# fkluger/vanishing_points_2017

Measured on AMD Instinct MI355X. Metric: images/sec (LSD->CNN->EM) + horizon-AUC parity, YUD-shape, 1/2/4/8 GPU, higher is better.
Workload: dtype f32 (CNN: f32 operands / accumulation / results; conv1 multiply EXACT bf16 pieces of the f32 operands (three per operand) on the bf16 matrix cores; conv2-5, fc6 and fc7 multiply scaled fp16 PAIRS of the f32 operands (22 of 24 significand bits, three exact products per f32 product) on the fp16 matrix

## Files before the change

### __graft_entry__.py

```python
import os
import subprocess
import sys

ROOT = os.path.dirname(os.path.abspath(__file__))
if ROOT not in sys.path:
    sys.path.insert(0, ROOT)


def build():
    from vanishing_points_2017_amd import build as vbuild
    so = vbuild.build(verbose=True)
    sim = os.path.join(ROOT, "tests", "hostsim")
    out = os.path.join(sim, "_build")
    os.makedirs(out, exist_ok=True)
    subprocess.check_call(["g++", "-O2", "-std=c++17", "-ffp-contract=off", "-fPIC", "-shared",
                           "-Wno-unknown-pragmas", os.path.join(sim, "sim_em.cpp"), "-o",
                           os.path.join(out, "libvpk_hostsim.so")])
    subprocess.check_call(["g++", "-O2", "-std=c++17", "-ffp-contract=off", "-fPIC", "-shared",
                           os.path.join(sim, "sim_raster.cpp"), "-o", os.path.join(out, "libvpk_hostsim_raster.so")])
    subprocess.check_call(["g++", "-O2", "-std=c++17", "-Wall", "-Werror", "-fPIC", "-shared",
                           os.path.join(sim, "sim_cnn_plan.cpp"), "-o", os.path.join(out, "libvpk_hostsim_cnn_plan.so")])
    odir = os.path.join(ROOT, "oracle", "_build")
    os.makedirs(odir, exist_ok=True)
    subprocess.check_call(["gcc", "-O2", "-fPIC", "-shared", "-ffp-contract=off", "-fno-builtin",
                           os.path.join(ROOT, "oracle", "_fma.c"), "-o", os.path.join(odir, "libvpkfma.so"), "-lm"])
    import vanishing_points_2017_amd
    from vanishing_points_2017_amd import _lib
    lib = _lib.load()
    missing = [s for s in _lib.EXPORTS if not hasattr(lib, s)]
    if missing:
        raise RuntimeError("libvpk.so lacks symbols: %s" % missing)
    print("built", so)


def smoke():
    import numpy as np
    import torch
    assert torch.cuda.is_available(), "smoke() needs cuda:0"
    from vanishing_points_2017_amd import synth, vp_localisation
    from oracle import em_numpy
    from oracle import agg_raster
    from vanishing_points_2017_amd import sphere_mapping
    sc = synth.make_scene(4242, 90, 3)
    ln = sc["l"]
    sc["sphere_image"] = sphere_mapping.sphere_line_plot(ln.copy(), 500, alpha=0.1)
    assert np.array_equal(sc["sphere_image"], agg_raster.raster(ln)), "the sphere raster differs from the oracle"
    got = vp_localisation.expectation_maximisation(sc["l"].copy(), sc["lp"].copy(), sc["cnn_response"],
                                                   sphere_image=sc["sphere_image"])
    ref = em_numpy.expectation_maximisation(sc["l"].copy(), sc["lp"].copy(), sc["cnn_response"].copy(),
                                            sphere_image=sc["sphere_image"])
    assert np.array_equal(got["vp_assoc"], ref["vp_assoc"]), "line->VP assignments differ from the oracle"
    assert np.abs(got["vp"] - ref["vp"]).max() < 1e-4
    from oracle import cnn_torch
    from vanishing_points_2017_amd import cnn
    w, mean = cnn.synthetic_weights(0), cnn.synthetic_mean(0)
    sphere = sc["sphere_image"][None]
    want = cnn_torch.forward(w, mean, sphere)
    net = cnn.Net(w, mean)
    err = []
    for alg in (4, 2):
        net.set_algorithm(alg)
        err.append(float(np.abs(net.forward(sphere) - want).max()))
    net.set_algorithm(4)
    assert max(err) <= 2e-5, "CNN response differs from the oracle: %s" % err
    print("smoke ok: raster of %d lines exact; %d VPs, %d iterations; CNN max |diff| %.1e (default: fp16 pairs) / %.1e (exact bf16 triples + Winograd f32)" % (
        ln.shape[0], got["vp"].shape[0], got["iterations"], err[0], err[1]))


if __name__ == "__main__":
    build()
    if len(sys.argv) > 1 and sys.argv[1] == "smoke":
        smoke()
```

### vanishing_points_2017_amd/cnn.py

```python
import ctypes

import numpy as np

from ._lib import VPK_ERR_RANGE, VpkRangeError
from .runtime import get_runtime

LAYER_SHAPES = [
    ("conv1", (96, 1, 11, 11)), ("conv2", (256, 48, 5, 5)), ("conv3", (384, 256, 3, 3)),
    ("conv4", (384, 192, 3, 3)), ("conv5", (256, 192, 3, 3)), ("fc6", (4096, 57600)),
    ("fc7", (4096, 4096)), ("fc8", (400, 4096)),
]
RANGE_POLICIES = {"raise": 0, "recompute_exact": 1}


def range_policy_code(policy):
    if policy not in RANGE_POLICIES:
        raise ValueError("range policy must be one of %s, got %r" % (sorted(RANGE_POLICIES), policy))
    return RANGE_POLICIES[policy]


FLOAT_DTYPES = ("float16", "float32", "float64")


def image_kind(images):
# ... 51 lines not shown
            if w.shape != shape or b.shape != (shape[0],):
                raise ValueError("%s: expected weight %s / bias (%d,), got %s / %s" % (name, shape, shape[0], w.shape, b.shape))
            keep += [w, b]
            blobs += [w.ctypes.data, b.ctypes.data]
        mean = np.ascontiguousarray(np.asarray(mean, dtype=np.float32).reshape(500, 500))
        arr = (ctypes.c_void_p * 16)(*blobs)
        self.rt.check(self.rt.lib.vpk_cnn_load(self.rt.h, arr, ctypes.c_void_p(mean.ctypes.data)))
        self._last_batch = None

    def forward_device(self, sphere, tap=None):
        f32 = image_kind(sphere) == "f32"
        if f32 and len(sphere.shape) != 3:
            raise ValueError("forward_device: float images must be (B, 500, 500), got shape %s" % (tuple(sphere.shape),))
        rt = self.rt
        t = rt.torch
        batch = int(sphere.shape[0])
        if f32 and sphere.is_cuda:
            rt.stream.wait_stream(t.cuda.current_stream(sphere.device))
        with rt.on_stream():
            if f32:
                sphere = sphere.to(device=rt.tdev, dtype=t.float32).contiguous()
            out = t.empty((batch, 20, 20), dtype=t.float32, device=rt.tdev)
            if tap is None:
                fwd = rt.lib.vpk_cnn_forward_f32 if f32 else rt.lib.vpk_cnn_forward
                rt.check(fwd(rt.h, rt.ptr(sphere), batch, rt.ptr(out)))
                self._last_batch = batch
                return out
            tp = t.empty((batch,) + TAP_SHAPES[tap], dtype=t.float32, device=rt.tdev)
            fwd = rt.lib.vpk_cnn_forward_tap_f32 if f32 else rt.lib.vpk_cnn_forward_tap
            rt.check(fwd(rt.h, rt.ptr(sphere), batch, rt.ptr(out), int(tap), rt.ptr(tp)))
            return out, tp

    LAYER_NAMES = ["conv1", "norm1", "pool1", "conv2", "norm2", "pool2", "conv3", "conv4", "conv5", "pool5",
                   "fc6", "fc7", "fc8"]
    LAYER_FLOP = {"conv1": 2 * 96 * 15129 * 121, "conv2": 2 * 256 * 3721 * 1200, "conv3": 2 * 384 * 900 * 2304,
                  "conv4": 2 * 384 * 900 * 1728, "conv5": 2 * 256 * 900 * 1728, "fc6": 2 * 57600 * 4096,
                  "fc7": 2 * 4096 * 4096, "fc8": 2 * 4096 * 400}

    @classmethod
    def executed_flop(cls, layer, fusion=3, precision=0, algorithm=4, batch=102):
        alg = cls.LAYER_FLOP[layer]
        if layer == "conv1":
            if fusion == 3:
                return 168 * 12 * 72 * 2.0 * 16 * 16 * 32, "bf16"
            if fusion == 4:
                return 168 * 12 * 48 * 2.0 * 16 * 16 * 32, "f16"
            if fusion == 1:
                return 168 * 8 * 186 * 2.0 * 16 * 16 * 4, "f32"
            return alg * 128.0 / 121.0, "f32"
        if layer in ("conv2", "conv3", "conv4", "conv5"):
            if precision == 1:
                return 6.0 * alg, "bf16"
            if algorithm == 4:
                tiles, steps = {"conv2": (2 * 16 * 2 * 1, 75), "conv3": (1 * 8 * 1 * 3, 16 * 9), "conv4": (2 * 4 * 1 * 3, 12 * 9),
                                "conv5": (2 * 8 * 1 * 1, 12 * 9)}[layer]
                return tiles * steps * 4 * 12 * 2.0 * 32 * 32 * 16, "f16"
            if layer == "conv2" and algorithm >= 2:
                return 64 * 4 * 75 * 24 * 2.0 * 32 * 32 * 16, "bf16"
            if algorithm >= 1:
                return alg * (36.0 / 100.0 if layer == "conv2" else 16.0 / 36.0), "f32"
            return alg, "f32"
        pad = (-(-batch // 128) * 128) / float(batch)
        if precision == 0 and ((layer == "fc6" and algorithm >= 2) or (layer == "fc7" and algorithm == 4)):
            return alg * pad * (3.0 if algorithm == 4 else 6.0), "f16" if algorithm == 4 else "bf16"
        return alg * pad, "f32"

    def set_fusion(self, on=3):
        self.rt.check(self.rt.lib.vpk_cnn_set_fusion(self.rt.h, int(on)))

    def set_algorithm(self, mode):
        self.rt.check(self.rt.lib.vpk_cnn_set_algorithm(self.rt.h, int(mode)))

    def set_precision(self, mode):
        self.rt.check(self.rt.lib.vpk_cnn_set_precision(self.rt.h, int(mode)))

    RANGE_LAYERS = ["conv2", "conv3", "conv4", "conv5", "fc6", "fc7"]

    def activation_scales(self):
        sc = (ctypes.c_float * 6)()
        self.rt.check(self.rt.lib.vpk_cnn_get_activation_scales(self.rt.h, sc))
        return np.array([float(x) for x in sc], dtype=np.float32)

    def set_activation_scales(self, scales):
        sc = (ctypes.c_float * 6)(*[float(x) for x in scales])
        self.rt.check(self.rt.lib.vpk_cnn_set_activation_scales(self.rt.h, sc))

    def calibrate(self, rasters=None):
        rt = self.rt
        if rasters is None:
            rt.check(rt.lib.vpk_cnn_calibrate(rt.h, None, 0))
            return
        t = rt.torch
        if not isinstance(rasters, t.Tensor):
            rasters = t.from_numpy(np.ascontiguousarray(rasters, dtype=np.uint8).reshape(-1, 500, 500))
        with rt.on_stream():
            d = rasters.to(rt.tdev).contiguous()
        rt.synchronize()
        rt.check(rt.lib.vpk_cnn_calibrate(rt.h, rt.ptr(d), int(d.shape[0])))

    def range_flags(self):
        w = ctypes.c_uint32(0)
        rc = self.rt.lib.vpk_cnn_range_flags(self.rt.h, ctypes.byref(w))
        if rc not in (0, VPK_ERR_RANGE):
            self.rt.check(rc)
        return int(w.value)

    def check_range(self):
        w = ctypes.c_uint32(0)
        rc = self.rt.lib.vpk_cnn_range_flags(self.rt.h, ctypes.byref(w))
# ... 94 lines not shown
```

### vanishing_points_2017_amd/csrc/cnn_conv_pieces.hpp

```cpp
#ifndef VPK_CNN_CONV_PIECES_HPP_
#define VPK_CNN_CONV_PIECES_HPP_

namespace {

constexpr int CP_THREADS = 256;
constexpr int CP_TC = 32;

struct PieceDims {
    int B;
    int Cg16, CGtot, Hp, Wp;
    int OC, OH, OW, groups;
    int KW, ntaps, ksteps;
    int mblocks;
    int mtiles, rtiles, ctiles;
    int relu;
    int OHp, OWp, opad;
    long long in_image;
    int o_cgtot, o_Hp, o_Wp, o_pad;
    float o_ascale;
    unsigned* range_word;
    unsigned range_bit;
    unsigned* img_range;
    const int* live;
    float oscale;
};


template <int NP>
__global__ __launch_bounds__(256) void to_planes_kernel(const float* __restrict__ in, unsigned short* __restrict__ out, int C, int Hp,
                                                        int Wp, float ascale, unsigned* __restrict__ range_word, unsigned range_bit,
                                                        unsigned* __restrict__ img_range, const int* __restrict__ live) {
    const int y = blockIdx.x, cg = blockIdx.y, b = blockIdx.z;
    if (live && b >= *live) return;
    const float* src = in + (((size_t)b * C + cg * 16) * Hp + y) * Wp;
    u32x4* dst = reinterpret_cast<u32x4*>(out) + (((size_t)b * (C >> 4) + cg) * (2 * NP) * Hp + y) * Wp;
    bool bad = false;
    for (int idx = threadIdx.x; idx < 2 * Wp; idx += 256) {
        const int h = idx / Wp, x = idx - h * Wp;
        unsigned short p[3][8];
#pragma unroll
        for (int e = 0; e < 8; ++e) {
            const float v = src[(size_t)(8 * h + e) * Hp * Wp + x];
            if (NP == 3) split3(v, p[0][e], p[1][e], p[2][e]);
            else split2h_guard(v * ascale, p[0][e], p[1][e], bad);
        }
#pragma unroll
        for (int q = 0; q < NP; ++q) {
            u32x4 w4;
#pragma unroll
            for (int e = 0; e < 4; ++e) w4[e] = (unsigned)p[q][2 * e] | ((unsigned)p[q][2 * e + 1] << 16);
            dst[(size_t)(2 * q + h) * Hp * Wp + x] = w4;
        }
    }
    if (NP == 2) range_report(bad, range_word, range_bit, img_range ? img_range + b : nullptr);
}

template <int N>
__device__ __forceinline__ void cp_wait() {
    asm volatile("s_waitcnt vmcnt(%0)" ::"n"(N) : "memory");
    __builtin_amdgcn_sched_barrier(0);
}

template <int OFF>
__device__ __forceinline__ void cp_gload16(bf16x8& dst, const void* sbase, unsigned voff) {
    asm volatile("global_load_dwordx4 %0, %1, %2 offset:%3" : "+v"(dst) : "v"(voff), "s"(sbase), "n"(OFF) : "memory");
}

template <int KH, int NB, int NP, int RH>
__global__ __launch_bounds__(CP_THREADS, 2) void conv_pieces_kernel(PieceDims d, const unsigned short* __restrict__ act,
                                                                     const unsigned short* __restrict__ wfrag,
                                                                     const float* __restrict__ bias, float* __restrict__ out,
                                                                     unsigned short* __restrict__ out_planes,
                                                                     int* __restrict__ tile_counter, int total_tiles) {
    constexpr int MB = 4 / RH;
    constexpr int TR = RH * NB;
    constexpr int PR = TR + KH - 1, PC = CP_TC + KH - 1;
    constexpr int KPP = (PC + 7) / 8;
    constexpr int PARTS = PR > 8 ? 2 : 1;
    constexpr int GST = (PR > 8 ? PR * 128 : 1024) + 128;
    static_assert(GST % 256 == 128, "odd multiple of 128 bytes");
    if (d.live) {
        d.B = __builtin_amdgcn_readfirstlane(*d.live);
        total_tiles = d.groups * d.B * d.rtiles * d.ctiles * d.mtiles;
    }
    constexpr int PLANE = KPP * GST;
    constexpr int NPL = 2 * NP;
    constexpr int PBUF = NPL * PLANE;
    constexpr int NDMA = NPL * KPP * PARTS;
    constexpr int NPW = (NDMA + 3) / 4;
    constexpr int NPR = NP == 3 ? 6 : 3;
    constexpr int NSETS = NP == 3 ? 2 : (KH == 5 ? 5 : (RH == 2 ? 6 : 3));
    constexpr int D = NSETS;
    constexpr int KHB = KH == 5 ? 5 : 1;
    constexpr int FP = KH == 5 ? 5 : 9;
    constexpr int NPWB = (NPW + KHB - 1) / KHB;
    static_assert(PR <= 16 && NB == 4 && (RH == 1 || RH == 2) && KH * KH == KHB * FP && (NP == 2 || NP == 3), "8 row slots per DMA instruction; two halves");
    __shared__ __attribute__((aligned(16))) unsigned char cp_lds[2 * PBUF];
    __shared__ int s_next[2];
    const int tid = threadIdx.x, lane = tid & 63;
    const int wave = __builtin_amdgcn_readfirstlane(tid >> 6);
    const int wmq = RH == 1 ? wave : (wave & 1);
    const int rh = RH == 1 ? 0 : (wave >> 1);
    const int n31 = lane & 31, kh_ = lane >> 5;
    const unsigned lds0 = lds_addr(cp_lds);
    typedef __attribute__((address_space(3))) const bf16x8 lds_cbf8;
    unsigned vb[KH];
#pragma unroll
    for (int kw = 0; kw < KH; ++kw) {
        const unsigned c = (unsigned)(n31 + kw);
        vb[kw] = lds0 + (unsigned)(kh_ * PLANE + rh * NB * 128) + (c >> 3) * (unsigned)GST + (c & 7u) * 16u;
    }
    const unsigned voff_a = (unsigned)lane * 16u;
    int parity = 0;
    for (int tile = blockIdx.x; tile < total_tiles;) {
        int nx = 0;
        if (tid == 0)
            asm volatile("s_nop 4\n\tglobal_atomic_add %0, %1, %2, %3 sc0" : "=v"(nx) : "v"(0), "v"(1), "s"(tile_counter) : "memory");
        int t = tile;
        const int mt = t % d.mtiles; t /= d.mtiles;
        const int ct = t % d.ctiles; t /= d.ctiles;
        const int rt = t % d.rtiles; t /= d.rtiles;
        const int b = t % d.B;
        const int g = t / d.B;
        const int y0 = rt * TR, x0 = ct * CP_TC;
        const unsigned char* in_g = reinterpret_cast<const unsigned char*>(act) + (size_t)b * d.in_image +
                                    (size_t)g * d.Cg16 * NPL * d.Hp * d.Wp * 16;
        const size_t plane_bytes = (size_t)d.Hp * d.Wp * 16;
        const int yr = y0 + (lane >> 3) < d.Hp ? y0 + (lane >> 3) : d.Hp - 1;
        const unsigned voff_p = (unsigned)(yr * d.Wp + x0 + (lane & 7)) * 16u;
        const int yr2 = y0 + 8 + (lane >> 3) < d.Hp ? y0 + 8 + (lane >> 3) : d.Hp - 1;
        const unsigned voff_p2 = (unsigned)(yr2 * d.Wp + x0 + (lane & 7)) * 16u;
        auto issue_dma = [&](int cg, int k) __attribute__((always_inline)) {
            int q = wave * NPW + k;
            q = q < NDMA ? q : NDMA - 1;
            const int part = q / (NPL * KPP), q1 = q - part * (NPL * KPP);
            const int pl = q1 / KPP, kk = q1 - pl * KPP;
            const unsigned char* src = in_g + ((size_t)cg * NPL + pl) * plane_bytes + (size_t)kk * 128;
            const unsigned dst = lds0 + (unsigned)((cg & 1) * PBUF + pl * PLANE + kk * GST);
            if (PARTS == 1 || part == 0) dma16(voff_p, src, __builtin_amdgcn_readfirstlane(dst));
            else if (lane < 8 * (PR - 8)) dma16(voff_p2, src, __builtin_amdgcn_readfirstlane(dst + 1024u));
        };
        const unsigned char* wgrp = reinterpret_cast<const unsigned char*>(wfrag) +
                                    ((size_t)g * d.ksteps * d.mblocks + (size_t)mt * MB + wmq) * NP * 1024;
        const unsigned wstep = (unsigned)d.mblocks * NP * 1024;
        bf16x8 af[NSETS][NP], bfr[NB][NP];
#pragma unroll
        for (int q = 0; q < NSETS * NP; ++q) af[q / NP][q % NP] = __builtin_bit_cast(bf16x8, u32x4{0u, 0u, 0u, 0u});
        auto load_a = [&](const unsigned char* src, auto o_tag) __attribute__((always_inline)) {
            constexpr int o = decltype(o_tag)::value;
            cp_gload16<0>(af[o][0], src, voff_a);
            cp_gload16<1024>(af[o][1], src, voff_a);
            if constexpr (NP == 3) cp_gload16<2048>(af[o][2], src, voff_a);
        };
        auto fetch_b = [&](auto row_tag, auto k_tag, unsigned va) __attribute__((always_inline)) {
            constexpr int j = decltype(row_tag)::value, k = decltype(k_tag)::value;
            constexpr int dkh = KH == 5 ? 0 : k / KH;
#pragma unroll
            for (int p = 0; p < NP; ++p) bfr[j][p] = *(lds_cbf8*)(va + (unsigned)((j + dkh) * 128 + p * 2 * PLANE));
        };
        auto tap_address = [&](auto k_tag, unsigned sb) __attribute__((always_inline)) {
            constexpr int k = decltype(k_tag)::value;
            return vb[KH == 5 ? k : k % KH] + sb;
        };
        auto fetch_all = [&](auto k_tag, unsigned sb) __attribute__((always_inline)) {
            const unsigned va = tap_address(k_tag, sb);
            fetch_b(std::integral_constant<int, 0>(), k_tag, va); fetch_b(std::integral_constant<int, 1>(), k_tag, va);
            fetch_b(std::integral_constant<int, 2>(), k_tag, va); fetch_b(std::integral_constant<int, 3>(), k_tag, va);
        };
        f32x2v acc[NB][8];
        f32x16 tq[NB];
#pragma unroll
        for (int j = 0; j < NB; ++j) {
#pragma unroll
            for (int e = 0; e < 8; ++e) acc[j][e] = f32x2v{0.f, 0.f};
#pragma unroll
            for (int e = 0; e < 16; ++e) tq[j][e] = 0.f;
        }
        const int S = d.ksteps;
        __builtin_amdgcn_s_barrier();
#pragma unroll
        for (int k = 0; k < NPW; ++k) issue_dma(0, k);
        asm volatile("s_nop 4" ::: "memory");
        load_a(wgrp, std::integral_constant<int, 0>());
        load_a(wgrp + wstep, std::integral_constant<int, 1>());
        if constexpr (NSETS > 2) load_a(wgrp + 2 * wstep, std::integral_constant<int, 2>());
        if constexpr (NSETS > 3) { load_a(wgrp + 3 * wstep, std::integral_constant<int, 3>()); load_a(wgrp + 4 * wstep, std::integral_constant<int, 4>()); }
        if constexpr (NSETS > 5) load_a(wgrp + 5 * wstep, std::integral_constant<int, 5>());
        const unsigned char* anext = wgrp + (size_t)D * wstep;
        cp_wait<0>();
        if (tid == 0) s_next[parity] = nx + (int)gridDim.x;
        asm volatile("s_waitcnt lgkmcnt(0)" ::: "memory");
        __builtin_amdgcn_s_barrier();
        fetch_all(std::integral_constant<int, 0>(), 0u);
        auto products = [&](auto o_tag, auto row_tag, auto first_tag) __attribute__((always_inline)) {
            constexpr int o = decltype(o_tag)::value, j = decltype(row_tag)::value;
            constexpr bool first = decltype(first_tag)::value;
            constexpr int PA[6] = {NP == 3 ? 2 : 1, NP == 3 ? 1 : 0, 0, 1, 0, 0}, PB[6] = {0, 1, NP == 3 ? 2 : 0, 0, 1, 0};
            const f32x16 zero = {0.f, 0.f, 0.f, 0.f, 0.f, 0.f, 0.f, 0.f, 0.f, 0.f, 0.f, 0.f, 0.f, 0.f, 0.f, 0.f};
#pragma unroll
            for (int p = 0; p < NPR; ++p) {
                if constexpr (NP == 3)
                    tq[j] = __builtin_amdgcn_mfma_f32_32x32x16_bf16(af[o][PA[p]], bfr[j][PB[p]], first && p == 0 ? zero : tq[j], 0, 0, 0);
                else
                    tq[j] = __builtin_amdgcn_mfma_f32_32x32x16_f16(__builtin_bit_cast(f16x8, af[o][PA[p]]), __builtin_bit_cast(f16x8, bfr[j][PB[p]]),
                                                                   first && p == 0 ? zero : tq[j], 0, 0, 0);
            }
        };
        auto fold_row = [&](auto row_tag) __attribute__((always_inline)) {
            constexpr int j = decltype(row_tag)::value;
            asm volatile("s_nop 7" ::: "memory");
#pragma unroll
            for (int e = 0; e < 8; ++e) {
                const f32x2v t2 = {tq[j][2 * e], tq[j][2 * e + 1]};
                f32x2v& a2 = acc[j][e];
                asm volatile("v_pk_add_f32 %0, %0, %1" : "+v"(a2) : "v"(t2));
            }
        };
        int kb = 0, cg = 0;
        auto step = [&](auto o_tag, auto k_tag, bool gs, bool dma_block, bool dma_prev, bool more_blocks, bool tail, unsigned sb) __attribute__((always_inline)) {
            constexpr int k = decltype(k_tag)::value;
            constexpr bool last = k + 1 == FP;
            constexpr int AHEAD = NP * (D - 1), AHEAD_TAIL = NP * (FP - 1 - k < D - 1 ? FP - 1 - k : D - 1);
            const bool dma_out = (k >= 1 && k <= D) ? dma_block : (k == 0 && D == FP ? dma_prev && !gs : false);
            if (tail) cp_wait<AHEAD_TAIL>();
            else if (dma_out) cp_wait<AHEAD + NPWB>();
            else cp_wait<AHEAD>();
            if (k == 0 && gs) {
                __builtin_amdgcn_s_barrier();
                fetch_all(k_tag, sb);
            }
            const unsigned va_next = k + 1 < FP ? tap_address(std::integral_constant<int, (k + 1 < FP ? k + 1 : 0)>(), sb)
                                                : tap_address(std::integral_constant<int, 0>(), sb + 128u);
#define CP_ROW(J)                                                                                                      \
            __builtin_amdgcn_sched_barrier(0);                                                                             \
            products(o_tag, std::integral_constant<int, J>(), std::integral_constant<bool, k == 0>());                     \
            __builtin_amdgcn_sched_barrier(0);                                                                             \
            if constexpr (k + 1 < FP) fetch_b(std::integral_constant<int, J>(), std::integral_constant<int, k + 1>(), va_next); \
            else if (more_blocks) fetch_b(std::integral_constant<int, J>(), std::integral_constant<int, 0>(), va_next);    \
            if constexpr (last && J > 0) fold_row(std::integral_constant<int, (J > 0 ? J - 1 : 0)>());                     \
            __builtin_amdgcn_sched_barrier(0);
            CP_ROW(0) CP_ROW(1) CP_ROW(2) CP_ROW(3)
#undef CP_ROW
            if (k < FP - D || !tail) { load_a(anext, o_tag); anext += wstep; }
            if (k == 0 && dma_block) {
#pragma unroll
                for (int i = 0; i < NPWB; ++i) issue_dma(cg + 1, kb * NPWB + i < NPW ? kb * NPWB + i : NPW - 1);
            }
            if constexpr (last) { asm volatile("s_nop 15" ::: "memory"); fold_row(std::integral_constant<int, NB - 1>()); }
            __builtin_amdgcn_sched_barrier(0);
        };
        bool dma_prev = false;
        auto block = [&](auto a_tag) __attribute__((always_inline)) {
            constexpr int a = decltype(a_tag)::value;
            const bool gs = kb == 0 && cg > 0;
            const bool dma_block = cg + 1 < d.Cg16 && kb * NPWB < NPW;
            const bool more = kb + 1 < KHB;
            const unsigned sb = (unsigned)((cg & 1) * PBUF + kb * 128);
            const bool tail = !more && cg + 1 == d.Cg16;
            static_assert(FP == 5 || FP == 9, "the steps of a block are written out for 5 and 9");
            static_assert(NP == 3 || (2 * FP) % NSETS == 0, "two blocks must be a whole number of set rotations");
#define CP_STEP(n) step(std::integral_constant<int, (NP == 3 ? (a + n) & 1 : (a + n) % NSETS)>(), std::integral_constant<int, n>(), gs, dma_block, dma_prev, more, tail, sb);
            CP_STEP(0) CP_STEP(1) CP_STEP(2) CP_STEP(3) CP_STEP(4)
            if constexpr (FP == 9) { CP_STEP(5) CP_STEP(6) CP_STEP(7) CP_STEP(8) }
#undef CP_STEP
            dma_prev = dma_block;
            if (++kb == KHB) { kb = 0; ++cg; }
        };
        const int nblocks = S / FP;
        if constexpr (NP == 3) {
            int bi = 0;
            for (; bi + 2 <= nblocks; bi += 2) {
                block(std::integral_constant<int, 0>());
                block(std::integral_constant<int, FP & 1>());
            }
            if (bi < nblocks) block(std::integral_constant<int, 0>());
        } else if constexpr (FP % NSETS == 0) {
            for (int bi = 0; bi < nblocks; ++bi) block(std::integral_constant<int, 0>());
        } else {
            int bi = 0;
            for (; bi + 2 <= nblocks; bi += 2) {
                block(std::integral_constant<int, 0>());
                block(std::integral_constant<int, FP % NSETS>());
            }
            if (bi < nblocks) block(std::integral_constant<int, 0>());
        }
        {
            int te = tile;
            unsigned le = voff_a;
            asm volatile("" : "+s"(te), "+v"(le));
            const int e_mt = te % d.mtiles; te /= d.mtiles;
            const int e_ct = te % d.ctiles; te /= d.ctiles;
            const int e_rt = te % d.rtiles; te /= d.rtiles;
            const int e_b = te % d.B, e_g = te / d.B;
            const int e_n31 = (int)(le >> 4) & 31, e_kh = (int)(le >> 9);
            const int ow = e_ct * CP_TC + e_n31;
            const int m_blk = (e_mt * MB + wmq) * 32;
            const unsigned plane = (unsigned)(d.OHp * d.OWp);
            const unsigned char* obase = reinterpret_cast<const unsigned char*>(out + ((size_t)e_b * d.groups + e_g) * d.OC * plane);
            const int oh0 = e_rt * TR + rh * NB;
            const unsigned vo0 = ((unsigned)(4 * e_kh) * plane + (unsigned)((oh0 + d.opad) * d.OWp + ow + d.opad)) * 4u;
            f32x4v bl[4];
#pragma unroll
            for (int q = 0; q < 4; ++q) {
                const int m0 = m_blk + 8 * q < d.OC ? m_blk + 8 * q : d.OC - 8;
                bl[q] = *reinterpret_cast<const f32x4v*>(bias + e_g * d.OC + m0 + 4 * e_kh);
            }
            if (NP == 2 && out_planes) {
                unsigned char* pbase = reinterpret_cast<unsigned char*>(out_planes) + (size_t)e_b * d.o_cgtot * 4 * d.o_Hp * d.o_Wp * 16;
                bool bad = false;
                const unsigned wplane = (unsigned)(d.o_Hp * d.o_Wp) * 16u;
                const unsigned vo_p = (unsigned)((oh0 + d.o_pad) * d.o_Wp + ow + d.o_pad) * 16u + 8u * (unsigned)e_kh;
#pragma unroll
                for (int j = 0; j < NB; ++j) {
                    if (ow >= d.OW || oh0 + j >= d.OH) continue;
#pragma unroll
                    for (int q = 0; q < 4; ++q) {
                        const int m0 = __builtin_amdgcn_readfirstlane(m_blk + 8 * q);
                        if (m0 >= d.OC) continue;
                        const int c0 = e_g * d.OC + m0;
                        unsigned short h0[4], h1[4];
#pragma unroll
                        for (int e = 0; e < 4; ++e) {
                            float v = acc[j][2 * q + e / 2][e % 2] * d.oscale + bl[q][e];
                            if (d.relu) v = v > 0.f ? v : 0.f;
                            split2h_guard(v * d.o_ascale, h0[e], h1[e], bad);
                        }
                        const unsigned w0 = ((unsigned)(c0 >> 4) * 4u + (unsigned)((c0 >> 3) & 1)) * wplane + vo_p + (unsigned)(j * d.o_Wp) * 16u;
                        *reinterpret_cast<u32x2*>(pbase + w0) = u32x2{(unsigned)h0[0] | ((unsigned)h0[1] << 16), (unsigned)h0[2] | ((unsigned)h0[3] << 16)};
                        *reinterpret_cast<u32x2*>(pbase + (w0 + 2u * wplane)) = u32x2{(unsigned)h1[0] | ((unsigned)h1[1] << 16), (unsigned)h1[2] | ((unsigned)h1[3] << 16)};
                    }
                }
                range_report(bad, d.range_word, d.range_bit, d.img_range ? d.img_range + e_b : nullptr);
            } else
#pragma unroll
            for (int j = 0; j < NB; ++j) {
                if (ow >= d.OW || oh0 + j >= d.OH) continue;
                const unsigned vo = vo0 + (unsigned)(j * d.OWp) * 4u;
#pragma unroll
                for (int q = 0; q < 4; ++q) {
                    const int m0 = __builtin_amdgcn_readfirstlane(m_blk + 8 * q);
                    if (m0 >= d.OC) continue;
#pragma unroll
// ... 16 lines not shown
```

### vanishing_points_2017_amd/csrc/cnn_plan.hpp

```cpp
#ifndef VPK_CNN_PLAN_HPP_
#define VPK_CNN_PLAN_HPP_

#include "../../include/vpk.h"

struct CnnConfig {
    int precision = 0;
    int split_variant = 0;
    int algorithm = 4;
    int fusion = 3;
    int conv1_group = 4;
    int dense_presplit = 1;
    bool profiling = false;
};

inline void cnn_config_set_precision(CnnConfig& c, int mode) {
    c.precision = mode ? 1 : 0;
    c.split_variant = mode > 1 ? mode - 1 : 0;
}

enum class Conv1Impl { GEMM, DIRECT_F32, GEMM_FUSED, PIECES3, PIECES2 };
enum class ConvImpl { DMA_F32, SPLIT_GEMM, WINOGRAD, PIECES3, PIECES2 };
enum class DenseImpl { DMA_F32, PIECES3, PIECES2_STREAMED, PIECES2_PRESPLIT };

struct ConvStage {
    ConvImpl impl = ConvImpl::DMA_F32;
    int split_tiling = 0;
    bool chained_in = false;
    bool chained_out = false;
    bool needs_to_planes = false;
    bool writes_next_planes = false;
};

struct CnnPlan {
    int err = VPK_OK;
    const char* msg = nullptr;
    bool prep_input = false;
    Conv1Impl conv1 = Conv1Impl::PIECES3;
    bool conv1_hands_planes = false;
    ConvStage conv[4];
    bool norm2_planes = false;
    bool norm2_hands_planes = false;
    DenseImpl fc[3] = {DenseImpl::DMA_F32, DenseImpl::DMA_F32, DenseImpl::DMA_F32};
};

inline CnnPlan cnn_resolve_plan(const CnnConfig& c, int tap, bool f32_images, bool device_counted) {
    CnnPlan p;
    const bool f32_mfma = c.precision == 0;
    const bool pairs = f32_mfma && c.algorithm == 4;
    const bool triples = f32_mfma && c.algorithm >= 2 && !pairs;
    const bool wino = f32_mfma && c.algorithm >= 1;
    const bool split = c.precision == 1;

    if (tap == 0 || c.fusion == 0) p.conv1 = Conv1Impl::GEMM;
    else if (c.fusion == 1) p.conv1 = Conv1Impl::DIRECT_F32;
    else if (c.fusion == 2) p.conv1 = Conv1Impl::GEMM_FUSED;
    else p.conv1 = c.fusion == 4 ? Conv1Impl::PIECES2 : Conv1Impl::PIECES3;
    p.prep_input = p.conv1 == Conv1Impl::GEMM || p.conv1 == Conv1Impl::GEMM_FUSED;
    const bool conv1_pieces = p.conv1 == Conv1Impl::PIECES3 || p.conv1 == Conv1Impl::PIECES2;
    p.conv1_hands_planes = conv1_pieces && pairs && tap != 1;
    if (f32_images && p.conv1 == Conv1Impl::PIECES2) {
        p.err = VPK_ERR_STATE;
        p.msg = "vpk_cnn_forward_f32: vpk_cnn_set_fusion(4) takes uint8 rasters only";
    }

// ... 38 lines not shown
```

### vanishing_points_2017_amd/csrc/vpk_cnn.hip

```cpp
#include "vpk_internal.hpp"

#include <stdlib.h>
#include <string.h>
#include <type_traits>
#include <vector>

#include "cnn_plan.hpp"
#include "cnn_topology.hpp"
#include "cnn_gemm_f32.hpp"
#include "cnn_conv1_direct.hpp"
#include "cnn_norm_pool.hpp"

namespace {

#include "cnn_split_gemm.hpp"
#include "cnn_pairs.hpp"
#include "cnn_conv1_pieces.hpp"
#include "cnn_conv_pieces.hpp"
#include "cnn_norm_pool_planes.hpp"
#include "cnn_dense_pieces.hpp"
#include "cnn_winograd.hpp"

struct Layer {
    ConvDims d;
// ... 213 lines not shown
        const unsigned short* sp = src_split;
        if (!sp) {
            unsigned short* cv = reinterpret_cast<unsigned short*>(R[R_SPLIT]);
            hipLaunchKernelGGL(split_nhwc_kernel, dim3((unsigned)sd.Hp, (unsigned)batch), dim3(256),
                               (size_t)sd.Ctot * (sd.Wp + 1) * sizeof(float), st, src, cv, sd.Ctot, sd.Hp, sd.Wp);
            sp = cv;
        }
        const int ntiles = (sd.N + SG_BN - 1) / SG_BN;
        auto go = [&](auto kernel, int blk, int threads, int per_cu) {
            const int total = sd.groups * ntiles * (sd.mblocks / blk);
            hipLaunchKernelGGL(kernel, dim3((unsigned)std::min(total, per_cu * h->num_cu)), dim3(threads), 0, st, sd, sp, l.wsplit,
                               l.bias, dst, ctr + li, total);
        };
        if (sd.OC == 192) {
            if (dst_split) go(conv_gemm_split_kernel<2, 4, 3, 3, 2, true>, 6, 512, 1);
            else go(conv_gemm_split_kernel<2, 4, 3, 3, 2, false>, 6, 512, 1);
        } else if (tiling == 1) {
            if (dst_split) go(conv_gemm_split_kernel<2, 2, 2, 2, 2, true>, 4, 256, 2);
            else go(conv_gemm_split_kernel<2, 2, 2, 2, 2, false>, 4, 256, 2);
        } else {
            if (dst_split) go(conv_gemm_split_kernel<2, 4, 2, 3, 2, true>, 4, 512, 1);
            else go(conv_gemm_split_kernel<2, 4, 2, 3, 2, false>, 4, 512, 1);
        }
    };
    auto conv_wino = [&](int li, const float* src, float* dst) {
        if (li == 1) {
            Wino5Dims w5 = S->L[1].wd5;
            w5.tiles = batch * W5_TPI;
            const int total = w5.groups * w5.ocblocks * ((w5.tiles + W5_TB - 1) / W5_TB);
            hipLaunchKernelGGL(conv5x5_winograd_kernel, dim3((unsigned)std::min(total, h->num_cu)), dim3(W5_THREADS), 0, st, w5, src,
                               S->L[1].wino, S->L[1].bias, dst, ctr + 1, total);
            return;
        }
        WinoDims wd = S->L[li].wd;
        wd.tiles = batch * WG_TILES_PER_IMAGE;
        const int total = wd.groups * wd.ocblocks * ((wd.tiles + WG_TB - 1) / WG_TB);
        hipLaunchKernelGGL(conv3x3_winograd_kernel, dim3((unsigned)std::min(total, h->num_cu)), dim3(WG_THREADS), 0, st, wd, src,
                           S->L[li].wino, S->L[li].bias, dst, ctr + li, total, live);
    };
    auto to_p6 = [&](int li, bool pairs, const float* src, unsigned short* dst) {
        const ConvDims& d = S->L[li].d;
        const int C = d.IC * d.groups;
        if (pairs) hipLaunchKernelGGL(to_planes_kernel<2>, dim3((unsigned)d.Hp, (unsigned)(C / 16), (unsigned)batch), dim3(256), 0, st, src, dst, C, d.Hp, d.Wp,
                                      S->L[li].ascale, fc.range_word, 1u << li, fc.img_range, live);
        else hipLaunchKernelGGL(to_planes_kernel<3>, dim3((unsigned)d.Hp, (unsigned)(C / 16), (unsigned)batch), dim3(256), 0, st, src, dst, C, d.Hp, d.Wp, 1.f,
                                fc.range_word, 0u, nullptr, live);
    };
    auto conv_pieces = [&](int li, bool pairs, const unsigned short* src6, float* dst, unsigned short* planes_next) {
        PieceDims pd = pairs ? S->L[li].pdh : S->L[li].pd;
        pd.B = batch;
        if (planes_next) { const PieceDims& nx = S->L[li + 1].pdh; pd.o_cgtot = nx.CGtot; pd.o_Hp = nx.Hp; pd.o_Wp = nx.Wp; pd.o_pad = 1; pd.o_ascale = S->L[li + 1].ascale; }
        pd.range_word = fc.range_word; pd.range_bit = 1u << (li + 1); pd.img_range = fc.img_range; pd.live = live;
        if (pairs) pd.oscale = 1.f / (S->L[li].hscale * S->L[li].ascale);
        constexpr int nb = 4;
        const int tile_rows = pairs && li == 3 ? 2 * nb : nb;
        pd.rtiles = (pd.OH + tile_rows - 1) / tile_rows;
        const int total = pd.groups * batch * pd.rtiles * pd.ctiles * pd.mtiles;
        const unsigned blocks = (unsigned)std::min(total, 2 * h->num_cu);
        auto go = [&](auto kernel) {
            hipLaunchKernelGGL(kernel, dim3(blocks), dim3(CP_THREADS), 0, st, pd, src6, pairs ? S->L[li].whalf : S->L[li].wsplit, S->L[li].bias,
                               dst, planes_next, ctr + li, total);
        };
        if (pairs) { if (li == 1) go(conv_pieces_kernel<5, nb, 2, 1>); else if (li == 3) go(conv_pieces_kernel<3, nb, 2, 2>); else go(conv_pieces_kernel<3, nb, 2, 1>); }
        else { if (li == 1) go(conv_pieces_kernel<5, nb, 3, 1>); else go(conv_pieces_kernel<3, nb, 3, 1>); }
    };
    auto conv_stage = [&](int li, const float* src, float* dst, unsigned short* planes, unsigned short* planes_next,
                          const unsigned short* split_in, unsigned short* split_out) {
        const ConvStage& cs = plan.conv[li - 1];
        const bool pairs = cs.impl == ConvImpl::PIECES2;
        switch (cs.impl) {
        case ConvImpl::PIECES3:
        case ConvImpl::PIECES2:
            if (cs.needs_to_planes) to_p6(li, pairs, src, planes);
            conv_pieces(li, pairs, planes, dst, cs.writes_next_planes ? planes_next : nullptr);
            break;
        case ConvImpl::SPLIT_GEMM:
            conv_split(li, cs.split_tiling, src, cs.chained_in ? split_in : nullptr, cs.chained_out ? (void*)split_out : (void*)dst, cs.chained_out);
            break;
        case ConvImpl::WINOGRAD:
            conv_wino(li, src, dst);
            break;
        case ConvImpl::DMA_F32:
            if (li == 3) launch_dma(h, conv_gemm_dma_kernel<1, 4, 3, 1, false>, dims(3), 96, src, S->L[3], dst, 1, ctr + 3);
            else launch_dma(h, conv_gemm_dma_kernel<2, 2, 2, 2, false>, dims(li), 128, src, S->L[li], dst, 1, ctr + li);
            break;
        }
    };
    unsigned short* p6_2 = reinterpret_cast<unsigned short*>(R[R_P6_2]);
    unsigned short* p6_3 = reinterpret_cast<unsigned short*>(R[R_P6_3]);
    unsigned short* p6_5 = reinterpret_cast<unsigned short*>(R[R_P6_5]);
    unsigned short* s4 = reinterpret_cast<unsigned short*>(R[R_SPLIT4]);
    unsigned short* s5 = reinterpret_cast<unsigned short*>(R[R_SPLIT5]);
    conv_stage(1, R[R_POOL1], R[R_CONV2], p6_2, nullptr, nullptr, nullptr);
    mark(1);
    if ((rc = tapcopy(2, R[R_CONV2], A_CONV2))) return rc;
    if (plan.norm2_planes)
        hipLaunchKernelGGL((lrn5_pool3s2_planes_kernel<6>), dim3((unsigned)(batch * 5 * 8)), dim3(256), 0, st, R[R_CONV2], R[R_POOL2],
                           plan.norm2_hands_planes ? p6_3 : nullptr, 256, 61, 61, 30, 30, 1e-4f, 32, 32, 1, 8,
                           S->L[2].ascale, fc.range_word, 1u << 2, fc.img_range);
    else
        hipLaunchKernelGGL((lrn5_pool3s2_stream_kernel<6, 4>), dim3((unsigned)(batch * 5 * 8)), dim3(256), 0, st, R[R_CONV2], R[R_POOL2],
                           256, 61, 61, 30, 30, 1e-4f, 0.75f, 32, 32, 1, 8, live);
    mark(2);
    tapunpad(3, R[R_POOL2], 256, 30, 30, 1);
    conv_stage(2, R[R_POOL2], R[R_CONV3], p6_3, p6_5, nullptr, s4);
    mark(1);
    tapunpad(4, R[R_CONV3], 384, 30, 30, 1);
    conv_stage(3, R[R_CONV3], R[R_CONV4], p6_5, p6_3, s4, s5);
    mark(1);
    tapunpad(5, R[R_CONV4], 384, 30, 30, 1);
    conv_stage(4, R[R_CONV4], R[R_CONV5], plan.conv[2].writes_next_planes ? p6_3 : p6_5, nullptr, s5, nullptr);
    mark(1);
    if ((rc = tapcopy(6, R[R_CONV5], A_CONV5))) return rc;
    hipLaunchKernelGGL((pool5_kernel<8>), dim3((unsigned)(((long long)batch * 256 + 7) / 8)), dim3(256), 0, st, R[R_CONV5], R[R_POOL5],
                       (long long)batch * 256, live);
    mark(1);
// ... 32 lines not shown
                break;
            case DenseImpl::PIECES2_STREAMED:
                hipLaunchKernelGGL(dense_pieces_kernel<2>, grid, dim3(DP_THREADS), 0, st, dd, S->L[li].wraw, S->xfrag, R[R_PART], ctr + li, total);
                break;
            default:
                hipLaunchKernelGGL(dense_pieces_kernel<3>, grid, dim3(DP_THREADS), 0, st, dd, S->L[li].wraw, S->xfrag, R[R_PART], ctr + li, total);
                break;
            }
            d.ksplit = dd.kparts;
        }
        const long long tot = (long long)d.N * d.OC;
        float* dst = li == 7 ? out : fc_out;
        float* pre = (li == 7 && tap == 10) ? tap_out : nullptr;
        hipLaunchKernelGGL(splitk_reduce_kernel, dim3(ew_blocks(tot)), dim3(256), 0, st, R[R_PART], S->L[li].bias, d.ksplit,
                           d.N, d.OC, li == 7 ? 2 : 1, dst, pre, live);
        mark(1);
        if (li == 5 && (rc = tapcopy(8, fc_out, A_FC6))) return rc;
        if (li == 6 && (rc = tapcopy(9, fc_out, A_FC7))) return rc;
        fc_in = fc_out;
        fc_out = (li == 5) ? R[R_FCB] : R[R_FCA];
    }
    if (cfg.profiling) {
        S->ev_valid = (evi == 14);
        if (S->ev_valid) ++S->ev_pass;
    }
    VPK_HIP(h, hipGetLastError());
    return VPK_OK;
}

}
#include "cnn_calibrate.hpp"
#include "cnn_range_policy.hpp"

namespace {

struct ScopedDeviceBuffer {
    void* p = nullptr;
    ~ScopedDeviceBuffer() { if (p) (void)hipFree(p); }
};

template <typename T>
int upload(vpk_handle* h, T** dst, const T* src, size_t n) {
    VPK_HIP(h, hipMalloc((void**)dst, n * sizeof(T)));
    VPK_HIP(h, hipMemcpy(*dst, src, n * sizeof(T), hipMemcpyHostToDevice));
    return VPK_OK;
}

int load_model(vpk_handle* h, const float* const blobs[16], const float* mean) {
    vpk_cnn_state* S = h->cnn;
    int rc;
    if ((rc = upload(h, &S->mean, mean, (size_t)500 * 500))) return rc;
    if (const char* e = getenv("VPK_CONV1_GROUP")) { const int v = atoi(e); if (v >= 1 && v <= 64) S->cfg.conv1_group = v; }
    if (const char* e = getenv("VPK_DENSE_PRESPLIT")) S->cfg.dense_presplit = atoi(e) != 0;
    for (int li = 0; li < 8; ++li) {
        const Topo& t = TOPO[li];
        const float* w = blobs[2 * li];
        Layer& l = S->L[li];
        ConvDims& d = l.d;
        d.B = 0; d.IC = t.IC; d.Hp = t.H + 2 * t.P; d.Wp = t.W + 2 * t.P; d.OC = t.OC; d.OH = t.OH; d.OW = t.OW; d.groups = t.G;
        d.OHp = t.OH + 2 * t.OP; d.OWp = t.OW + 2 * t.OP; d.opad = t.OP;
        if (li == 0) { d.IC = C1_PH * C1_PH; d.Hp = C1_PW; d.Wp = C1_PW; }
        d.K = t.IC * t.KH * t.KH;
        d.Kp = (d.K + BK - 1) / BK * BK;
        d.Mp = (t.OC + t.BM - 1) / t.BM * t.BM;
        d.N = 0;
        d.ksplit = KSPLIT[li];
        d.relu = 1;
        const size_t w_floats = (size_t)t.G * t.OC * d.K;
        const size_t p_floats = (size_t)t.G * d.Kp * d.Mp;
        {
            ScopedDeviceBuffer rawbuf;
            VPK_HIP(h, hipMalloc(&rawbuf.p, w_floats * sizeof(float)));
            const float* raw = static_cast<const float*>(rawbuf.p);
            VPK_HIP(h, hipMemcpy(rawbuf.p, w, w_floats * sizeof(float), hipMemcpyHostToDevice));
            VPK_HIP(h, hipMalloc((void**)&l.wp, p_floats * sizeof(float)));
            hipLaunchKernelGGL(pack_weights_kernel, dim3((unsigned)((p_floats + 255) / 256)), dim3(256), 0, h->stream, raw,
                               l.wp, t.G, t.OC, d.K, d.Kp, d.Mp);
            VPK_HIP(h, hipStreamSynchronize(h->stream));
            if (li == 5 || li == 6) {
                const int chunks = d.K / DP_CHUNK, mtiles = (t.OC + DP_BM - 1) / DP_BM;
                const long long total4 = (long long)mtiles * chunks * DP_BM * (DP_CHUNK / 4);
                VPK_HIP(h, hipMalloc((void**)&l.wraw, (size_t)total4 * 16));
                hipLaunchKernelGGL(dense_tile_weights_kernel, dim3((unsigned)((total4 + 255) / 256)), dim3(256), 0, h->stream, raw, l.wraw, t.OC, d.K,
                                   chunks, total4);
                VPK_HIP(h, hipStreamSynchronize(h->stream));
                l.hscale = weight_scale_pow2(w, w_floats);
                const long long total16 = (long long)mtiles * chunks * 8 * 2 * 2 * 64;
                VPK_HIP(h, hipMalloc((void**)&l.wpair, (size_t)total16 * 16));
                hipLaunchKernelGGL(dense_pair_weights_kernel, dim3((unsigned)((total16 + 255) / 256)), dim3(256), 0, h->stream, raw, l.wpair, t.OC,
                                   d.K, chunks, l.hscale, total16);
                VPK_HIP(h, hipStreamSynchronize(h->stream));
            }
        }
        if (li < 5) {
            std::vector<unsigned> tab(d.Kp, 0u);
            for (int k = 0; k < d.K; ++k) {
                int ic = k / (t.KH * t.KH), r = k % (t.KH * t.KH), kh = r / t.KH, kw = r % t.KH;
                if (li == 0)
                    tab[k] = (unsigned)((((kh % C1_PH) * C1_PH + kw % C1_PH) * C1_PW + kh / C1_PH) * C1_PW + kw / C1_PH) * 4u;
                else
                    tab[k] = (unsigned)((ic * d.Hp + kh) * d.Wp + kw) * 4u;
            }
            if ((rc = upload(h, &l.ktab, tab.data(), tab.size()))) return rc;
        }
        if (li >= 1 && li <= 4) {
            SplitDims& sd = l.sd;
// ... 283 lines not shown
```

Measured before the change: 23020.

## Skip dead output rows in edge conv tiles and schedule edge tiles last

Adds an EDGE template parameter to the pieces convolution kernel so tiles at the bottom image edge issue fetches and MFMA products only for output rows that exist, choosing a reduced-row instantiation at runtime. For 3x3 layers it also reorders the persistent tile queue so all edge row-tiles run after the full tiles, which is meant to balance the load at the end of the queue. This removes wasted matrix-core work on padded rows but adds more code paths per kernel, which raises instruction footprint and register pressure. It is controlled by a new env knob that is on by default.

```diff
diff --git a/__graft_entry__.py b/__graft_entry__.py
--- a/__graft_entry__.py
+++ b/__graft_entry__.py
@@ -20,6 +20,8 @@
                            os.path.join(sim, "sim_raster.cpp"), "-o", os.path.join(out, "libvpk_hostsim_raster.so")])
     subprocess.check_call(["g++", "-O2", "-std=c++17", "-Wall", "-Werror", "-fPIC", "-shared",
                            os.path.join(sim, "sim_cnn_plan.cpp"), "-o", os.path.join(out, "libvpk_hostsim_cnn_plan.so")])
+    subprocess.check_call(["g++", "-O2", "-std=c++17", "-Wall", "-Werror", "-fPIC", "-shared",
+                           os.path.join(sim, "sim_cnn_tile_order.cpp"), "-o", os.path.join(out, "libvpk_hostsim_cnn_tile_order.so")])
     odir = os.path.join(ROOT, "oracle", "_build")
     os.makedirs(odir, exist_ok=True)
     subprocess.check_call(["gcc", "-O2", "-fPIC", "-shared", "-ffp-contract=off", "-fno-builtin",
diff --git a/vanishing_points_2017_amd/cnn.py b/vanishing_points_2017_amd/cnn.py
--- a/vanishing_points_2017_amd/cnn.py
+++ b/vanishing_points_2017_amd/cnn.py
@@ -127,9 +127,9 @@
             if precision == 1:
                 return 6.0 * alg, "bf16"
             if algorithm == 4:
-                tiles, steps = {"conv2": (2 * 16 * 2 * 1, 75), "conv3": (1 * 8 * 1 * 3, 16 * 9), "conv4": (2 * 4 * 1 * 3, 12 * 9),
-                                "conv5": (2 * 8 * 1 * 1, 12 * 9)}[layer]
-                return tiles * steps * 4 * 12 * 2.0 * 32 * 32 * 16, "f16"
+                blocks, rows, steps = {"conv2": (2 * 4 * 2, 61, 75), "conv3": (1 * 12 * 1, 30, 16 * 9), "conv4": (2 * 6 * 1, 30, 12 * 9),
+                                       "conv5": (2 * 4 * 1, 30, 12 * 9)}[layer]
+                return blocks * rows * steps * 3 * 2.0 * 32 * 32 * 16, "f16"
             if layer == "conv2" and algorithm >= 2:
                 return 64 * 4 * 75 * 24 * 2.0 * 32 * 32 * 16, "bf16"
             if algorithm >= 1:
diff --git a/vanishing_points_2017_amd/csrc/cnn_conv_pieces.hpp b/vanishing_points_2017_amd/csrc/cnn_conv_pieces.hpp
--- a/vanishing_points_2017_amd/csrc/cnn_conv_pieces.hpp
+++ b/vanishing_points_2017_amd/csrc/cnn_conv_pieces.hpp
@@ -1,5 +1,7 @@
 #ifndef VPK_CNN_CONV_PIECES_HPP_
 #define VPK_CNN_CONV_PIECES_HPP_
+
+#include "cnn_tile_order.hpp"
 
 namespace {
 
@@ -23,6 +25,7 @@
     unsigned* img_range;
     const int* live;
     float oscale;
+    int edge;
 };
 
 
@@ -66,7 +69,7 @@
     asm volatile("global_load_dwordx4 %0, %1, %2 offset:%3" : "+v"(dst) : "v"(voff), "s"(sbase), "n"(OFF) : "memory");
 }
 
-template <int KH, int NB, int NP, int RH>
+template <int KH, int NB, int NP, int RH, int EDGE = NB>
 __global__ __launch_bounds__(CP_THREADS, 2) void conv_pieces_kernel(PieceDims d, const unsigned short* __restrict__ act,
                                                                      const unsigned short* __restrict__ wfrag,
                                                                      const float* __restrict__ bias, float* __restrict__ out,
@@ -94,6 +97,8 @@
     constexpr int KHB = KH == 5 ? 5 : 1;
     constexpr int FP = KH == 5 ? 5 : 9;
     constexpr int NPWB = (NPW + KHB - 1) / KHB;
+    static_assert(EDGE >= 1 && EDGE <= NB, "live rows of an edge tile's last wave");
+    constexpr bool LAST = EDGE < NB && KH == 3;
     static_assert(PR <= 16 && NB == 4 && (RH == 1 || RH == 2) && KH * KH == KHB * FP && (NP == 2 || NP == 3), "8 row slots per DMA instruction; two halves");
     __shared__ __attribute__((aligned(16))) unsigned char cp_lds[2 * PBUF];
     __shared__ int s_next[2];
@@ -116,13 +121,14 @@
         int nx = 0;
         if (tid == 0)
             asm volatile("s_nop 4\n\tglobal_atomic_add %0, %1, %2, %3 sc0" : "=v"(nx) : "v"(0), "v"(1), "s"(tile_counter) : "memory");
-        int t = tile;
+        int t = LAST && d.edge == 1 ? cp_tile_order(tile, d.ctiles * d.mtiles, d.rtiles, d.groups * d.B) : tile;
         const int mt = t % d.mtiles; t /= d.mtiles;
         const int ct = t % d.ctiles; t /= d.ctiles;
         const int rt = t % d.rtiles; t /= d.rtiles;
         const int b = t % d.B;
         const int g = t / d.B;
         const int y0 = rt * TR, x0 = ct * CP_TC;
+        const int live_rows = d.edge ? (d.OH - (y0 + rh * NB) < NB ? (d.OH - (y0 + rh * NB) > 0 ? d.OH - (y0 + rh * NB) : 0) : NB) : NB;
         const unsigned char* in_g = reinterpret_cast<const unsigned char*>(act) + (size_t)b * d.in_image +
                                     (size_t)g * d.Cg16 * NPL * d.Hp * d.Wp * 16;
         const size_t plane_bytes = (size_t)d.Hp * d.Wp * 16;
@@ -162,10 +168,13 @@
             constexpr int k = decltype(k_tag)::value;
             return vb[KH == 5 ? k : k % KH] + sb;
         };
-        auto fetch_all = [&](auto k_tag, unsigned sb) __attribute__((always_inline)) {
+        auto fetch_all = [&](auto lr_tag, auto k_tag, unsigned sb) __attribute__((always_inline)) {
+            constexpr int LR = decltype(lr_tag)::value;
             const unsigned va = tap_address(k_tag, sb);
-            fetch_b(std::integral_constant<int, 0>(), k_tag, va); fetch_b(std::integral_constant<int, 1>(), k_tag, va);
-            fetch_b(std::integral_constant<int, 2>(), k_tag, va); fetch_b(std::integral_constant<int, 3>(), k_tag, va);
+            if constexpr (LR > 0) fetch_b(std::integral_constant<int, 0>(), k_tag, va);
+            if constexpr (LR > 1) fetch_b(std::integral_constant<int, 1>(), k_tag, va);
+            if constexpr (LR > 2) fetch_b(std::integral_constant<int, 2>(), k_tag, va);
+            if constexpr (LR > 3) fetch_b(std::integral_constant<int, 3>(), k_tag, va);
         };
         f32x2v acc[NB][8];
         f32x16 tq[NB];
@@ -191,7 +200,6 @@
         if (tid == 0) s_next[parity] = nx + (int)gridDim.x;
         asm volatile("s_waitcnt lgkmcnt(0)" ::: "memory");
         __builtin_amdgcn_s_barrier();
-        fetch_all(std::integral_constant<int, 0>(), 0u);
         auto products = [&](auto o_tag, auto row_tag, auto first_tag) __attribute__((always_inline)) {
             constexpr int o = decltype(o_tag)::value, j = decltype(row_tag)::value;
             constexpr bool first = decltype(first_tag)::value;
@@ -217,28 +225,35 @@
             }
         };
         int kb = 0, cg = 0;
-        auto step = [&](auto o_tag, auto k_tag, bool gs, bool dma_block, bool dma_prev, bool more_blocks, bool tail, unsigned sb) __attribute__((always_inline)) {
-            constexpr int k = decltype(k_tag)::value;
+        auto step = [&](auto lr_tag, auto o_tag, auto k_tag, bool gs, bool dma_block, bool dma_prev, bool more_blocks, bool tail, unsigned sb) __attribute__((always_inline)) {
+            constexpr int k = decltype(k_tag)::value, LR = decltype(lr_tag)::value;
             constexpr bool last = k + 1 == FP;
             constexpr int AHEAD = NP * (D - 1), AHEAD_TAIL = NP * (FP - 1 - k < D - 1 ? FP - 1 - k : D - 1);
             const bool dma_out = (k >= 1 && k <= D) ? dma_block : (k == 0 && D == FP ? dma_prev && !gs : false);
             if (tail) cp_wait<AHEAD_TAIL>();
             else if (dma_out) cp_wait<AHEAD + NPWB>();
             else cp_wait<AHEAD>();
+            if constexpr (LR == 0) {
+                constexpr int o = decltype(o_tag)::value;
+#pragma unroll
+                for (int p = 0; p < NP; ++p) asm volatile("" : "+v"(af[o][p]));
+            }
             if (k == 0 && gs) {
                 __builtin_amdgcn_s_barrier();
-                fetch_all(k_tag, sb);
+                fetch_all(lr_tag, k_tag, sb);
             }
             const unsigned va_next = k + 1 < FP ? tap_address(std::integral_constant<int, (k + 1 < FP ? k + 1 : 0)>(), sb)
                                                 : tap_address(std::integral_constant<int, 0>(), sb + 128u);
 #define CP_ROW(J)                                                                                                      \
+            if constexpr (J < LR) {                                                                                        \
             __builtin_amdgcn_sched_barrier(0);                                                                             \
             products(o_tag, std::integral_constant<int, J>(), std::integral_constant<bool, k == 0>());                     \
             __builtin_amdgcn_sched_barrier(0);                                                                             \
             if constexpr (k + 1 < FP) fetch_b(std::integral_constant<int, J>(), std::integral_constant<int, k + 1>(), va_next); \
             else if (more_blocks) fetch_b(std::integral_constant<int, J>(), std::integral_constant<int, 0>(), va_next);    \
             if constexpr (last && J > 0) fold_row(std::integral_constant<int, (J > 0 ? J - 1 : 0)>());                     \
-            __builtin_amdgcn_sched_barrier(0);
+            __builtin_amdgcn_sched_barrier(0);                                                                             \
+            }
             CP_ROW(0) CP_ROW(1) CP_ROW(2) CP_ROW(3)
 #undef CP_ROW
             if (k < FP - D || !tail) { load_a(anext, o_tag); anext += wstep; }
@@ -246,11 +261,11 @@
 #pragma unroll
                 for (int i = 0; i < NPWB; ++i) issue_dma(cg + 1, kb * NPWB + i < NPW ? kb * NPWB + i : NPW - 1);
             }
-            if constexpr (last) { asm volatile("s_nop 15" ::: "memory"); fold_row(std::integral_constant<int, NB - 1>()); }
+            if constexpr (last && LR > 0) { asm volatile("s_nop 15" ::: "memory"); fold_row(std::integral_constant<int, (LR > 0 ? LR - 1 : 0)>()); }
             __builtin_amdgcn_sched_barrier(0);
         };
         bool dma_prev = false;
-        auto block = [&](auto a_tag) __attribute__((always_inline)) {
+        auto block = [&](auto lr_tag, auto a_tag) __attribute__((always_inline)) {
             constexpr int a = decltype(a_tag)::value;
             const bool gs = kb == 0 && cg > 0;
             const bool dma_block = cg + 1 < d.Cg16 && kb * NPWB < NPW;
@@ -259,7 +274,7 @@
             const bool tail = !more && cg + 1 == d.Cg16;
             static_assert(FP == 5 || FP == 9, "the steps of a block are written out for 5 and 9");
             static_assert(NP == 3 || (2 * FP) % NSETS == 0, "two blocks must be a whole number of set rotations");
-#define CP_STEP(n) step(std::integral_constant<int, (NP == 3 ? (a + n) & 1 : (a + n) % NSETS)>(), std::integral_constant<int, n>(), gs, dma_block, dma_prev, more, tail, sb);
+#define CP_STEP(n) step(lr_tag, std::integral_constant<int, (NP == 3 ? (a + n) & 1 : (a + n) % NSETS)>(), std::integral_constant<int, n>(), gs, dma_block, dma_prev, more, tail, sb);
             CP_STEP(0) CP_STEP(1) CP_STEP(2) CP_STEP(3) CP_STEP(4)
             if constexpr (FP == 9) { CP_STEP(5) CP_STEP(6) CP_STEP(7) CP_STEP(8) }
 #undef CP_STEP
@@ -267,27 +282,38 @@
             if (++kb == KHB) { kb = 0; ++cg; }
         };
         const int nblocks = S / FP;
-        if constexpr (NP == 3) {
-            int bi = 0;
-            for (; bi + 2 <= nblocks; bi += 2) {
-                block(std::integral_constant<int, 0>());
-                block(std::integral_constant<int, FP & 1>());
-            }
-            if (bi < nblocks) block(std::integral_constant<int, 0>());
-        } else if constexpr (FP % NSETS == 0) {
-            for (int bi = 0; bi < nblocks; ++bi) block(std::integral_constant<int, 0>());
+        auto blocks = [&](auto lr_tag) __attribute__((always_inline)) {
+            fetch_all(lr_tag, std::integral_constant<int, 0>(), 0u);
+            if constexpr (NP == 3) {
+                int bi = 0;
+                for (; bi + 2 <= nblocks; bi += 2) {
+                    block(lr_tag, std::integral_constant<int, 0>());
+                    block(lr_tag, std::integral_constant<int, FP & 1>());
+                }
+                if (bi < nblocks) block(lr_tag, std::integral_constant<int, 0>());
+            } else if constexpr (FP % NSETS == 0) {
+                for (int bi = 0; bi < nblocks; ++bi) block(lr_tag, std::integral_constant<int, 0>());
+            } else {
+                int bi = 0;
+                for (; bi + 2 <= nblocks; bi += 2) {
+                    block(lr_tag, std::integral_constant<int, 0>());
+                    block(lr_tag, std::integral_constant<int, FP % NSETS>());
+                }
+                if (bi < nblocks) block(lr_tag, std::integral_constant<int, 0>());
+            }
+        };
+        if constexpr (EDGE == NB) {
+            blocks(std::integral_constant<int, NB>());
         } else {
-            int bi = 0;
-            for (; bi + 2 <= nblocks; bi += 2) {
-                block(std::integral_constant<int, 0>());
-                block(std::integral_constant<int, FP % NSETS>());
-            }
-            if (bi < nblocks) block(std::integral_constant<int, 0>());
+            if (live_rows > EDGE) blocks(std::integral_constant<int, NB>());
+            else if (RH == 2 && live_rows == 0) blocks(std::integral_constant<int, (RH == 2 ? 0 : EDGE)>());
+            else blocks(std::integral_constant<int, EDGE>());
         }
         {
             int te = tile;
             unsigned le = voff_a;
             asm volatile("" : "+s"(te), "+v"(le));
+            if (LAST && d.edge == 1) te = cp_tile_order(te, d.ctiles * d.mtiles, d.rtiles, d.groups * d.B);
             const int e_mt = te % d.mtiles; te /= d.mtiles;
             const int e_ct = te % d.ctiles; te /= d.ctiles;
             const int e_rt = te % d.rtiles; te /= d.rtiles;
diff --git a/vanishing_points_2017_amd/csrc/cnn_plan.hpp b/vanishing_points_2017_amd/csrc/cnn_plan.hpp
--- a/vanishing_points_2017_amd/csrc/cnn_plan.hpp
+++ b/vanishing_points_2017_amd/csrc/cnn_plan.hpp
@@ -10,6 +10,7 @@
     int fusion = 3;
     int conv1_group = 4;
     int dense_presplit = 1;
+    int conv_edge_rows = 1;
     bool profiling = false;
 };
 
diff --git a/vanishing_points_2017_amd/csrc/cnn_tile_order.hpp b/vanishing_points_2017_amd/csrc/cnn_tile_order.hpp
--- /dev/null
+++ b/vanishing_points_2017_amd/csrc/cnn_tile_order.hpp
@@ -0,0 +1,22 @@
+#ifndef VPK_CNN_TILE_ORDER_HPP_
+#define VPK_CNN_TILE_ORDER_HPP_
+
+#if defined(__HIPCC__)
+#define VPK_TILE_HD __host__ __device__
+#else
+#define VPK_TILE_HD
+#endif
+
+VPK_TILE_HD inline int cp_tile_order(int pos, int inner, int rtiles, int nimg) {
+    if (rtiles < 2) return pos;
+    const int full_per = (rtiles - 1) * inner;
+    const int nfull = nimg * full_per;
+    if (pos < nfull) {
+        const int q = pos / full_per;
+        return pos + q * inner;
+    }
+    const int e = pos - nfull, q = e / inner;
+    return e + (q + 1) * full_per;
+}
+
+#endif
diff --git a/vanishing_points_2017_amd/csrc/vpk_cnn.hip b/vanishing_points_2017_amd/csrc/vpk_cnn.hip
--- a/vanishing_points_2017_amd/csrc/vpk_cnn.hip
+++ b/vanishing_points_2017_amd/csrc/vpk_cnn.hip
@@ -289,6 +289,7 @@
         if (planes_next) { const PieceDims& nx = S->L[li + 1].pdh; pd.o_cgtot = nx.CGtot; pd.o_Hp = nx.Hp; pd.o_Wp = nx.Wp; pd.o_pad = 1; pd.o_ascale = S->L[li + 1].ascale; }
         pd.range_word = fc.range_word; pd.range_bit = 1u << (li + 1); pd.img_range = fc.img_range; pd.live = live;
         if (pairs) pd.oscale = 1.f / (S->L[li].hscale * S->L[li].ascale);
+        pd.edge = cfg.conv_edge_rows;
         constexpr int nb = 4;
         const int tile_rows = pairs && li == 3 ? 2 * nb : nb;
         pd.rtiles = (pd.OH + tile_rows - 1) / tile_rows;
@@ -298,7 +299,7 @@
             hipLaunchKernelGGL(kernel, dim3(blocks), dim3(CP_THREADS), 0, st, pd, src6, pairs ? S->L[li].whalf : S->L[li].wsplit, S->L[li].bias,
                                dst, planes_next, ctr + li, total);
         };
-        if (pairs) { if (li == 1) go(conv_pieces_kernel<5, nb, 2, 1>); else if (li == 3) go(conv_pieces_kernel<3, nb, 2, 2>); else go(conv_pieces_kernel<3, nb, 2, 1>); }
+        if (pairs) { if (li == 1) go(conv_pieces_kernel<5, nb, 2, 1, 1>); else if (li == 3) go(conv_pieces_kernel<3, nb, 2, 2, 2>); else go(conv_pieces_kernel<3, nb, 2, 1, 2>); }
         else { if (li == 1) go(conv_pieces_kernel<5, nb, 3, 1>); else go(conv_pieces_kernel<3, nb, 3, 1>); }
     };
     auto conv_stage = [&](int li, const float* src, float* dst, unsigned short* planes, unsigned short* planes_next,
@@ -437,6 +438,7 @@
     if ((rc = upload(h, &S->mean, mean, (size_t)500 * 500))) return rc;
     if (const char* e = getenv("VPK_CONV1_GROUP")) { const int v = atoi(e); if (v >= 1 && v <= 64) S->cfg.conv1_group = v; }
     if (const char* e = getenv("VPK_DENSE_PRESPLIT")) S->cfg.dense_presplit = atoi(e) != 0;
+    if (const char* e = getenv("VPK_CONV_EDGE_ROWS")) { const int v = atoi(e); if (v >= 0 && v <= 2) S->cfg.conv_edge_rows = v; }
     for (int li = 0; li < 8; ++li) {
         const Topo& t = TOPO[li];
         const float* w = blobs[2 * li];
```

Result: no change. 23140, median of 6 (+0.6%).
